# haotiansun14/rl-rep

Measured on AMD Instinct MI355X. Metric: gradient steps/sec (encoder+critic+actor) at batch=256, higher is better.
Workload: dtype f32

## Files before the change

rlrep_amd/csrc/engine.hip:

```cpp
#include "engine_internal.h"
#include <cstdarg>
#include <memory>

static thread_local char g_err[512] = "";
long long g_rl_launches = 0;
void rl_set_error(const char* fmt, ...) {
    va_list ap; va_start(ap, fmt); vsnprintf(g_err, sizeof(g_err), fmt, ap); va_end(ap);
}

static thread_local RlGrp g_grp;
static thread_local bool g_grp_on = false;
extern "C" const RlGrp* rl_grp_active() { return g_grp_on ? &g_grp : nullptr; }
struct GrpScope {
    bool set = false, prev_on = false; RlGrp prev{};
    explicit GrpScope(const rlrep_agent* ag) {
        if (!ag || ag->members <= 0) return;
        prev = g_grp; prev_on = g_grp_on;
        g_grp.members = ag->members; g_grp.stride = ag->grp_stride; g_grp.ring_stride = ag->grp_ring_stride; g_grp.seeds = ag->grp_seeds;
        g_grp_on = set = true;
    }
    ~GrpScope() { if (set) { g_grp = prev; g_grp_on = prev_on; } }
};
#define GROUP_REFUSE(what) \
    if (ag && ag->members > 0) { rl_set_error("%s: not available on a seed group (rlrep_group_create)", what); return RLREP_ERR_ARG; }
// ... 658 lines not shown
    };

    const std::vector<FinTask> cfins = {
        Builder::fin_sum(part_q + 0, nblk, 4, 1.0f / (float)B, ag->metrics + M_Q1_LOSS), Builder::fin_sum(part_q + 1, nblk, 4, 1.0f / (float)B, ag->metrics + M_Q2_LOSS),
        Builder::fin_sum(part_q + 2, nblk, 4, 1.0f / (float)B, ag->metrics + M_Q1), Builder::fin_sum(part_q + 3, nblk, 4, 1.0f / (float)B, ag->metrics + M_Q2)};
    const int ncdw_splits = rl_nc_dw_splits(B, F, H, 2);
    float* const ncdw_slab = ws.f((size_t)2 * ncdw_splits * H * F);
    float* const ncdw_bslab = ws.f((size_t)2 * ncdw_splits * H);
    const bool ncdw_in_adam = rl_nc_dw_engine() == 1 && ag->h.world_size <= 1 && ((H * F) & 3) == 0 && (H & 3) == 0 && ncdw_splits <= 16 && !rl_off("fold_ncdw");
    if (ncdw_in_adam) {
        const LT& w1 = ag->L.get("critic.l1.weight"); const LT& b1 = ag->L.get("critic.l1.bias");
        AdamTask::Slab sw; memset(&sw, 0, sizeof(sw));
        sw.off = w1.off - ag->L.group_off[1]; sw.n = 2ll * H * F; sw.per = (long long)H * F; sw.slab = ncdw_slab; sw.splits = ncdw_splits;
        AdamTask::Slab sb = sw;
        sb.off = b1.off - ag->L.group_off[1]; sb.n = 2ll * H; sb.per = H; sb.slab = ncdw_bslab;
        b.group_slabs[1] = {sw, sb};
    }
    auto critic_program = [&](Program& p, int hoist) {
        GemmTask tt[3], tn[3], tp[3];
        gauss_tasks(ag, !nft, fnet, s0.XF, SA, SA, gt, tt);
        gauss_tasks(ag, !nft, fnet, s0.XF2, SA, SA, gn, tn);
        gauss_tasks(ag, !nft, fnet, s0.XFpi, SA, SA, gp, tp);
        if (hoist == 2) {
            b.fwd_stage(p, {tt[0], tn[0], tp[0]}, "ft.l1(s,a) ft.l1(s',a') ft.l1(s,a_pi)");
            b.fwd_stage(p, {tt[1], tn[1], tp[1]}, "ft.l2 x3");
            b.fwd_stage(p, {tt[2], tn[2], tp[2]}, "ft.heads x3");
        } else if (hoist == 1) {
            b.fwd_stage(p, {actor_l(ag, 0, s0.XF2, SA, ab), actor_l(ag, 0, s0.XFpi, SA, ab_pi), tt[0]}, "actor.l1(s') actor.l1(s) ft.l1(s,a)");
            b.fwd_stage(p, {actor_l(ag, 1, nullptr, 0, ab), actor_l(ag, 1, nullptr, 0, ab_pi), tt[1]}, "actor.l2 x2 ft.l2");
            b.fwd_stage(p, {policy_head_task(ag, ab, s0.XF2 + S, SA, FLAG_DYN_EPS), policy_head_task(ag, ab_pi, s0.XFpi + S, SA, FLAG_DYN_EPS2), tt[2]},
                        "actor.head x2 ft.heads + policy");
            b.fwd_stage(p, {tn[0], tp[0]}, "ft.l1(s',a') ft.l1(s,a_pi)");
            b.fwd_stage(p, {tn[1], tp[1]}, "ft.l2 x2");
            b.fwd_stage(p, {tn[2], tp[2]}, "ft.heads x2");
        } else {
            b.fwd_stage(p, {actor_l(ag, 0, s0.XF2, SA, ab), tt[0]}, "actor.l1(s') ft.l1(s,a)");
            b.fwd_stage(p, {actor_l(ag, 1, nullptr, 0, ab), tt[1]}, "actor.l2 ft.l2");
            actor_head_stage(b, p, ag, ab, s0.XF2 + S, SA, {tt[2]}, "actor.head ft.heads + policy");
            b.fwd_stage(p, {tn[0]}, "ft.l1(s',a')");
            b.fwd_stage(p, {tn[1]}, "ft.l2");
            b.fwd_stage(p, {tn[2]}, "ft.heads");
        }
        {
            NcFwdTask live1 = nc_task(gt.HH, Pw("critic.l1.weight"), Pw("critic.l1.bias"), HmC, U, ag->W3("critic.l1.weight"));
            live1.sigma_out = SIG;
            nc_stage(p, {nc_task(gn.HH, Tw("critic_target.l1.weight"), Tw("critic_target.l1.bias"), HmT, nullptr, ag->W3("critic_target.l1.weight")),
                         nc_task(gn.HH, Tw("critic_target.l4.weight"), Tw("critic_target.l4.bias"), HmT + BH, nullptr, ag->W3("critic_target.l4.weight")),
                         live1,
                         nc_task(gt.HH, Pw("critic.l4.weight"), Pw("critic.l4.bias"), HmC + BH, U + BNH, ag->W3("critic.l4.weight"))}, "noise critic l1/l4 (target+live)");
        }
        b.fwd_stage(p, {Builder::fwd(HmT, H, B, H, Tw("critic_target.l2.weight"), H, Tw("critic_target.l2.bias"), H, Et, H, ACT_ELU),
                        Builder::fwd(HmT + BH, H, B, H, Tw("critic_target.l5.weight"), H, Tw("critic_target.l5.bias"), H, Et + BH, H, ACT_ELU),
                        Builder::fwd(HmC, H, B, H, Pw("critic.l2.weight"), H, Pw("critic.l2.bias"), H, Ec, H, ACT_ELU),
                        Builder::fwd(HmC + BH, H, B, H, Pw("critic.l5.weight"), H, Pw("critic.l5.bias"), H, Ec + BH, H, ACT_ELU)}, "critic l2/l5");
        QHeadCritic q; memset(&q, 0, sizeof(q));
        q.Et[0] = Et; q.Et[1] = Et + BH; q.Ec[0] = Ec; q.Ec[1] = Ec + BH;
        q.wt[0] = q.wt[1] = Tw("critic_target.l3.weight"); q.bt[0] = q.bt[1] = Tw("critic_target.l3.bias");
        q.wc[0] = q.wc[1] = Pw("critic.l3.weight"); q.bc[0] = q.bc[1] = Pw("critic.l3.bias");
        q.logp = ab.logp; q.R = s0.R; q.D = s0.D; q.alpha_state = ag->a.alpha_state_dev; q.gamma = ag->h.discount;
        q.inv_batch = ag->inv_batch(); q.dq = dq; q.GE[0] = GE; q.GE[1] = GE + BH; q.partial = part_q;
        q.B = B; q.H = H; q.nblk = nblk; q.train = 1; q.step = ag->adam_step + 1;
        p.stages.push_back({[=](hipStream_t st) { return rl_launch_qhead_critic(&q, st); }, "qhead critic"});
        b.dx_stage(p, {Builder::dx(GE, H, B, H, Pw("critic.l2.weight"), H, GHm, H, H, ACT_NONE, nullptr, 0),
                       Builder::dx(GE + BH, H, B, H, Pw("critic.l5.weight"), H, GHm + BH, H, H, ACT_NONE, nullptr, 0)}, "critic l2/l5 dx");
        b.dw_stage(p, {Builder::dw(dq, 1, 1, Ec, H, H, 2 * B, Gw("critic.l3.weight"), H, Gw("critic.l3.bias")),
                       Builder::dw(GE, H, H, HmC, H, H, B, Gw("critic.l2.weight"), H, Gw("critic.l2.bias")),
                       Builder::dw(GE + BH, H, H, HmC + BH, H, H, B, Gw("critic.l5.weight"), H, Gw("critic.l5.bias"))}, "critic dW l3 l2 l5");
        {
            NcDwBatch nb; memset(&nb, 0, sizeof(nb));
            nb.ntasks = 2;
            nb.lean = b.low_prio ? 1 : 0;
            int base_tile = 0;
            auto ncdw = [&](int q, float* Ubuf, float* GH, float* gW, float* gb) {
                NcDwTask& t = nb.t[q];
                t.U = Ubuf; t.GH = GH; t.ldgh = H; t.mean = gt.HH; t.sigma = SIG; t.ld_ml = 2 * F;
                t.noise = noise; t.gW = gW; t.gb = gb; t.B = B; t.F = F; t.H = H; t.N = N;
                t.tiles_k = (F + 31) / 32; t.ntiles = ((H + 15) / 16) * t.tiles_k; t.tile_base = base_tile; base_tile += t.ntiles;
            };
            ncdw(0, U, GHm, Gw("critic.l1.weight"), Gw("critic.l1.bias"));
            ncdw(1, U + BNH, GHm + BH, Gw("critic.l4.weight"), Gw("critic.l4.bias"));
            nb.splits = ncdw_splits; nb.slab = ncdw_slab; nb.bslab = ncdw_bslab;
            nb.engine = rl_nc_dw_engine();
            nb.fin_in_adam = ncdw_in_adam ? 1 : 0;
            if (nb.engine == 1) {
                base_tile = 0;
                for (int q = 0; q < 2; ++q) {
                    nb.t[q].ntiles = ((H + 63) / 64) * ((F + 63) / 64) * nb.splits; nb.t[q].tile_base = base_tile; base_tile += nb.t[q].ntiles;
                }
            }
            const int total = base_tile;
            p.stages.push_back({[=](hipStream_t st) { return rl_launch_nc_dw(&nb, total, st); }, "noise critic dW l1/l4"});
            Builder::tag(p, RLREP_ENGINE_NOISE_CRITIC, 2.0 * 2.0 * (double)B * N * F * H, 2.0 * 4.0 * ((double)B * N * H + (double)B * H + 2.0 * (double)B * F + (double)F * H));
        }
    };
    critic_program(ag->critic_bwd, 0);
    if (can_hoist) critic_program(ag->critic_bwd_h, 1);
    if (!ag->feat_bwd_h.stages.empty()) critic_program(ag->critic_bwd_h2, 2);
    b.adam(ag->critic_apply, 1, ag->h.lr_critic, nullptr, 0, 0, 0.f, cfins, "adam critic");
    critic_apply_folded(b, ag, "critic_target.l1.weight", cfins);

    auto actor_program = [&](Program& p, int& resume) {
        GemmTask tt[3];
        gauss_tasks(ag, !nft, fnet, s0.XFpi, SA, SA, gp, tt);
        b.fwd_stage(p, {actor_l(ag, 0, s0.XFpi, SA, ab_pi)}, "actor.l1(s)");
        b.fwd_stage(p, {actor_l(ag, 1, nullptr, 0, ab_pi)}, "actor.l2");
        actor_head_stage(b, p, ag, ab_pi, s0.XFpi + S, SA, {}, "actor.head + policy");
        b.fwd_stage(p, {tt[0]}, "ft.l1(s,a_pi)");
        b.fwd_stage(p, {tt[1]}, "ft.l2");
        b.fwd_stage(p, {tt[2]}, "ft.heads");
        resume = (int)p.stages.size();
        nc_stage(p, {nc_task(gp.HH, Pw("critic.l1.weight"), Pw("critic.l1.bias"), HmC, U, ag->W3("critic.l1.weight")),
                     nc_task(gp.HH, Pw("critic.l4.weight"), Pw("critic.l4.bias"), HmC + BH, U + BNH, ag->W3("critic.l4.weight"))}, "noise critic l1/l4");
        b.fwd_stage(p, {Builder::fwd(HmC, H, B, H, Pw("critic.l2.weight"), H, Pw("critic.l2.bias"), H, Ec, H, ACT_ELU),
                        Builder::fwd(HmC + BH, H, B, H, Pw("critic.l5.weight"), H, Pw("critic.l5.bias"), H, Ec + BH, H, ACT_ELU)}, "critic l2/l5");
        QHeadActor q; memset(&q, 0, sizeof(q));
        q.Ec[0] = Ec; q.Ec[1] = Ec + BH; q.wc[0] = q.wc[1] = Pw("critic.l3.weight"); q.bc[0] = q.bc[1] = Pw("critic.l3.bias");
        q.logp = ab_pi.logp; q.alpha_state = ag->a.alpha_state_dev; q.inv_batch = ag->inv_batch(); q.target_entropy = ag->h.target_entropy;
        q.GE[0] = GE; q.GE[1] = GE + BH; q.partial_loss = part_l; q.partial_c = ag->Gtail();
        q.B = B; q.H = H; q.nblk = nblk; q.step = ag->adam_step + 2;
        p.stages.push_back({[=](hipStream_t st) { return rl_launch_qhead_actor(&q, st); }, "qhead actor"});
        b.dx_stage(p, {Builder::dx(GE, H, B, H, Pw("critic.l2.weight"), H, GHm, H, H, ACT_NONE, nullptr, 0),
                       Builder::dx(GE + BH, H, B, H, Pw("critic.l5.weight"), H, GHm + BH, H, H, ACT_NONE, nullptr, 0)}, "critic l2/l5 dx");
        {
            NcDxTask t; memset(&t, 0, sizeof(t));
            t.GH[0] = GHm; t.GH[1] = GHm + BH; t.ldgh = H; t.U[0] = U; t.U[1] = U + BNH;
            t.W[0] = Pw("critic.l1.weight"); t.W[1] = Pw("critic.l4.weight"); t.noise = noise;
            t.lstd = gp.HH ? gp.HH + F : nullptr; t.ld_l = 2 * F; t.G = GTH; t.ldg = 2 * F;
            t.B = B; t.F = F; t.H = H; t.N = N; t.nheads = 2;
            t.tiles_k = (F + 63) / 64; t.ntiles = ((B + 3) / 4) * t.tiles_k; t.tile_base = 0;
            p.stages.push_back({[=](hipStream_t st) { return rl_launch_nc_dx(&t, st); }, "noise critic dX -> (dmean, dlog_std)"});
            Builder::tag(p, RLREP_ENGINE_NOISE_CRITIC, 2.0 * 2.0 * (double)B * N * F * H, 4.0 * (2.0 * ((double)B * N * H + (double)B * H + (double)F * H) + 3.0 * (double)B * F));
        }
        b.dx_stage(p, {Builder::dx(GTH, 2 * F, B, 2 * F, FT("mean_linear.weight"), Hv, GT2, Hv, Hv, ACT_RELU, gp.H2, Hv)}, "ft.heads dx");
        b.dx_stage(p, {Builder::dx(GT2, Hv, B, Hv, FT("l2.weight"), Hv, GT1, Hv, Hv, ACT_RELU, gp.H1, Hv)}, "ft.l2 dx");
        actor_backward(b, p, ag, ab_pi, s0.XFpi, SA, s0.XFpi + S, SA, Builder::dx(GT1, Hv, B, Hv, FT("l1.weight") ? FT("l1.weight") + S : nullptr, SA, ab_pi.dA, A, A, ACT_NONE, nullptr, 0));
    };
    actor_program(ag->actor_bwd, ag->actor_resume);
    actor_apply_program(b, ag, part_l, nblk);
    update_target_program(ag, "critic.l1.weight", "critic_target.l1.weight");

    for (int set = 0; set < rlrep_agent::NSETS; ++set) {
        const LT& f0 = ag->L.get(fnet + ".l1.weight");
        const LT& fl = ag->L.get(fnet + ".log_std_linear.bias");
        float* fbase = nft ? ag->a.param_dev : ag->a.target_dev;
        const Slot keep = defer_begin(b, ag, set, nft ? "f." : "f_target.", nft ? "f.l1.weight" : "f_target.l1.weight", fbase ? fbase + f0.off : nullptr,
                                      fl.off + fl.rows - f0.off);
        {
            rlrep_agent::DeferSet& D = ag->dset[set];
            const LT& p0 = ag->L.get("f.l1.weight");
            D.block_off = p0.off - ag->L.group_off[0]; D.block_n = fl.off + fl.rows - f0.off; D.block_which = nft ? 0 : 1;
            if (rl_off("fold_snapshot")) D.block_which = -1;
        }
        critic_program(ag->dset[set].critic_bwd, can_hoist ? 1 : 0);
        actor_program(ag->dset[set].actor_bwd, ag->dset[set].actor_resume);
        if (!can_hoist) ag->dset[set].actor_resume = 0;
        defer_end(b, ag, set, keep, "critic_target.l1.weight", cfins);
    }
}

Slot defer_begin(Builder& b, rlrep_agent* ag, int set, const char* prefix, const char* first, const float* block_src, int64_t block_n) {
    Workspace& ws = b.ws;
    const int B = ag->B, S = ag->d.state_dim, A = ag->d.action_dim, SA = S + A;
    Slot& s0 = ag->slot[0];
    rlrep_agent::DeferSet& D = ag->dset[set];
    Slot d; d.XE = nullptr; d.XF = ws.f((size_t)B * SA); d.XF2 = ws.f((size_t)B * SA); d.XFpi = ws.f((size_t)B * SA); d.R = ws.f(B); d.D = ws.f(B);
    D.slot = d;
// ... 1108 lines not shown
```

rlrep_amd/csrc/kparams.h:

```cpp
#pragma once
#include <stdint.h>
#include "dp_pull.h"
struct GroupCfg;

struct SlotFill {
    const float* ring; const int* idx;
    const float *s, *a, *r, *s2, *d;
    int B, S, A;
    float *XE, *XF, *XF2, *XFpi, *R, *D;
};

struct SelectAct {
    const float* obs; float* act;
    const float *W1, *b1, *W2, *b2, *W3, *b3;
    int S, Ha, A, explore;
    float lo, hi;
    unsigned long long seed, offset;
};
struct PhiloxFill {
    float* dst_f; int* dst_i; long long n;
    int kind;
    float std; int hi; const int* hi_dev;
    unsigned long long seed, offset; const int* step_dev; uint32_t stream_id;
    int step_add;
// ... 86 lines not shown
    if (g.in_a) g.in_a = (const float*)((uintptr_t)g.in_a + (uintptr_t)mdelta);
    if (g.in_b) g.in_b = (const float*)((uintptr_t)g.in_b + (uintptr_t)mdelta);
    if (g.alpha_state) g.alpha_state = (double*)((uintptr_t)g.alpha_state + (uintptr_t)mdelta);
    return g;
}
template <bool GRP = false>
__device__ inline void finalize_tasks(const FinTask* __restrict__ fin, int nfin, int lane, const DpPull* dp = nullptr, long long mdelta = 0) {
    for (int q = 0; q < nfin; ++q) {
        const FinTask f = fin_record<GRP>(fin[q], mdelta);
        if (f.kind == FIN_SUM) {
            float s = 0.f;
            for (int i = lane; i < f.count; i += 64) s += f.partials[(size_t)i * f.stride];
            s = wave_sum(s);
            if (lane == 0) *f.out = s * f.scale;
        } else if (f.kind == FIN_COMBINE) {
            if (lane == 0) *f.out = f.scale * (*f.in_a) + f.scale_b * (*f.in_b);
        } else if (f.kind == FIN_INC) {
            if (lane == 0) *reinterpret_cast<int*>(f.out) += 1;
        } else if (f.kind == FIN_COPY) {
            if (lane == 0) *f.out = *f.in_a;
        } else if (f.kind == FIN_ALPHA) {
            float s = 0.f;
            if (dp) {
                const long long toff = (long long)(f.partials - dp->base[dp->rank]);
                for (int i = lane; i < f.count; i += 64) s += dp_sum1(*dp, toff + (long long)i * f.stride);
            } else {
                for (int i = lane; i < f.count; i += 64) s += f.partials[(size_t)i * f.stride];
            }
            s = wave_sum(s);
            if (lane == 0) {
                double* st = f.alpha_state;
                const float mean_c = s * f.scale;
                const double alpha = exp(st[0]);
                *f.out = (float)alpha * mean_c;
                if (f.learn) {
                    const double g = (double)mean_c * alpha;
                    const double b1 = (double)f.beta1, b2 = (double)f.beta2;
                    st[3] += 1.0;
                    st[1] = st[1] + (1.0 - b1) * (g - st[1]);
                    st[2] = st[2] * b2 + (1.0 - b2) * g * g;
                    const double bc1 = 1.0 - pow(b1, st[3]), bc2 = 1.0 - pow(b2, st[3]);
                    const double denom = sqrt(st[2]) / sqrt(bc2) + (double)f.eps;
                    st[0] = st[0] - ((double)f.lr / bc1) * (st[1] / denom);
                }
                *f.out2 = (float)exp(st[0]);
            }
        } else if (f.kind == FIN_HISTORY) {
            __builtin_amdgcn_s_waitcnt(0x0F70);
            asm volatile("" ::: "memory");
            int* seq = reinterpret_cast<int*>(const_cast<float*>(f.partials));
            const int n = *seq;
            float* rec = f.out + (size_t)(n % f.count) * RL_HIST_REC;
            if (lane < f.stride) rec[lane] = __hip_atomic_load(f.in_a + lane, __ATOMIC_RELAXED, __HIP_MEMORY_SCOPE_AGENT);
            if (lane == RL_HIST_TAG) reinterpret_cast<int*>(rec)[RL_HIST_TAG] = n;
            if (lane == 0) *seq = n + 1;
        }
    }
}
#endif

struct NcFwdTask {
    const float* mean; const float* lstd; int ld_ml;
    const float* noise;
    const float* W; const float* bias;
    const unsigned char* W3;
    float* Hm;
    float* U;
    float* sigma_out;
    int B, F, H, N;
    int tiles_h, tile_base, ntiles;
};

#define NC_MAX_TASKS 4
struct NcFwdBatch { int ntasks; int engine; int cols; int nt_u; NcFwdTask t[NC_MAX_TASKS]; };

struct NcDwTask {
    const float* U; const float* GH; int ldgh;
    const float* mean; const float* sigma; int ld_ml;
    const float* noise;
    float* gW; float* gb;
    int B, F, H, N;
    int tiles_k, tile_base, ntiles;
};
struct NcDwBatch { int ntasks; int lean; int engine; int splits; float* slab; float* bslab; int fin_in_adam; int pad_; NcDwTask t[2]; };

struct NcDxTask {
    const float* GH[2]; int ldgh;
    const float* U[2];
    const float* W[2];
    const float* noise;
    const float* lstd; int ld_l;
    float* G; int ldg;
    int B, F, H, N, nheads;
    int tiles_k, tile_base, ntiles;
};


#define NC_NF_HOST 5

struct InfoNce {
    float* S; int ldS;
    int ncols, diag_off;
    const float* rhat; const float* r; float* drhat;
    float* partial; int B, nblk; float inv_batch; GroupCfg* step;
    const float* Z; int ldZ, F; const float* theta_w; const float* theta_b;
    const float* ZM; int ldZM;
};
struct ColSum { const float* X; int ldX; const float* w; float* out; int rows, F; const float* X2; int ldX2; const float* w2; float* out2; float* outb2; int rows2; DpSlots dp; };
#define RL_SLOTS_MAX_F 65536
struct SpederRows {
    const float* phi; const float* mu; const float* mu_r; const float* phibar;
    const float* theta_w; const float* theta_b; const float* r;
    float* c; float* drhat; float* partial; int B, F, nblk; float inv_batch; GroupCfg* step;
};
struct SpederGrads {
    const float* phi; const float* mu; const float* c; const float* drhat; const float* phibar; const float* v;
    const float* theta_w; float* Gphi; float* Gmu; int B, F; float inv_batch;
};
struct RegStats { const float* X[4]; const float* C[4]; int B, H, nbc, nbr; float lambda; float* partial; };

struct DiffsrPerturb {
    const float* alphabars; const int* idx; const float* s2; int ld_s2; const float* eps;
    float* XN; float* TGT; int B, S; GroupCfg* step0; GroupCfg* step1;
};
struct DiffsrScore {
    float* U; const float* PHI; const float* TGT; const float* alphabars; const int* idx;
    float* GPHI; float* partial; int B, F, S; float sigma, inv_batch;
};

enum XcKind : int { XC_GEMM = 0, XC_HEADS_VAE = 1, XC_QHEAD_CRITIC = 2, XC_QHEAD_ACTOR = 3 };
struct XcPhase {
    int kind;
    int task0, ntasks;
    int la, lb, vecA, vecB, pre;
    int tiles;
    int aux;
    int dyn;
    int rbg, R;
    int tb[GEMM_MAX_TASKS], tcs[GEMM_MAX_TASKS];
};
#define XC_GROUPS 8
#define XC_FLAG_STRIDE 64
struct XcLaunch {
    const XcPhase* ph; int nph;
    const GemmTask* tasks; const HeadsVae* hv; const QHeadCritic* qc; const QHeadActor* qa;
    int ntasks, nhv, nqc, nqa;
    unsigned* flags;
    unsigned* err;
    int rbg;
    int mpg;
    const float* dyn[3];
    int low_prio;
};
```

rlrep_amd/csrc/noisecritic.hip:

```cpp
#include <type_traits>
#include "common.h"
extern long long g_rl_launches;
#include "kparams.h"
#include "x3.h"

#define NC_NF 5

extern __shared__ __attribute__((aligned(16))) float nc_smem[];

#ifdef RL_TIMING_NC
__device__ unsigned long long g_nc_tim[6 * 4096];
extern "C" int rl_nc_timing_fetch(unsigned long long* host, int n) {
    return (int)hipMemcpyFromSymbol(host, HIP_SYMBOL(g_nc_tim), sizeof(unsigned long long) * n);
}
#define NCT(k) do { if (threadIdx.x == 0 && blockIdx.x < 4096) g_nc_tim[6 * blockIdx.x + (k)] = (k) < 4 ? clock64() : wall_clock64(); } while (0)
#else
#define NCT(k) do {} while (0)
#endif

__device__ __forceinline__ void ld4(const float* p, bool vec, int valid, float (&v)[4]) {
    if (vec && valid == 4) { f32x4 x = *reinterpret_cast<const f32x4*>(p); v[0] = x[0]; v[1] = x[1]; v[2] = x[2]; v[3] = x[3]; }
    else {
#pragma unroll
        for (int s = 0; s < 4; ++s) v[s] = (s < valid) ? p[s] : 0.f;
// ... 1182 lines not shown
            }
            if (want_bias) asum += (o.a[0] + o.a[1]) + (o.a[2] + o.a[3]);
        };
        const int nchunks = (Mb + 15) / 16;
        const int ngroups = (nchunks + 31) / 32;
        auto compg = [&](int g, const Chunk (&S)[4]) {
            const int c = w + 32 * g;
            Prep p0, p1;
            prep(c, S[0], p0);
            __builtin_amdgcn_sched_barrier(0);
            prep(c + 8, S[1], p1); mac(p0);
            __builtin_amdgcn_sched_barrier(0);
            prep(c + 16, S[2], p0); mac(p1);
            __builtin_amdgcn_sched_barrier(0);
            prep(c + 24, S[3], p1); mac(p0);
            __builtin_amdgcn_sched_barrier(0);
            mac(p1);
        };
        if constexpr (LEAN) {
            for (int g = 0; g < ngroups; g += 2) {
                __builtin_amdgcn_sched_barrier(0);
                if (g + 2 < ngroups) {
                    compg(g, S0);     loadg(g + 2, S0); __builtin_amdgcn_sched_barrier(0);
                    compg(g + 1, S1); loadg(g + 3, S1);
                } else {
                    compg(g, S0);
                    if (g + 1 < ngroups) compg(g + 1, S1);
                }
            }
        } else
        for (int g = 0; g < ngroups; g += 4) {
            __builtin_amdgcn_sched_barrier(0);
            if (g + 4 < ngroups) {
                compg(g, S0);     loadg(g + 4, S0); __builtin_amdgcn_sched_barrier(0);
                compg(g + 1, S1); loadg(g + 5, S1); __builtin_amdgcn_sched_barrier(0);
                compg(g + 2, S2); loadg(g + 6, S2); __builtin_amdgcn_sched_barrier(0);
                compg(g + 3, S3); loadg(g + 7, S3);
            } else {
                compg(g, S0);
                if (g + 1 < ngroups) compg(g + 1, S1);
                if (g + 2 < ngroups) compg(g + 2, S2);
                if (g + 3 < ngroups) compg(g + 3, S3);
            }
        }
    }
#pragma unroll
    for (int f = 0; f < 2; ++f)
#pragma unroll
        for (int r = 0; r < 4; ++r) red[w][f][r][lane] = acc[f][r];
    if (want_bias) {
        asum += __shfl_xor(asum, 16, 64);
        asum += __shfl_xor(asum, 32, 64);
        if (lane < 16) bsum[w][lane] = asum;
    }
    __syncthreads();
    {
        const int ol = threadIdx.x & 63, q = threadIdx.x >> 6;
        const int f = q >> 2, r = q & 3;
        float v = 0.f;
#pragma unroll
        for (int ww = 0; ww < 8; ++ww) v += red[ww][f][r][ol];
        const int row = j0 + (ol >> 4) * 4 + r, colk = k0 + 16 * f + (ol & 15);
        if (row < H && colk < F) {
            const size_t o = (size_t)row * F + colk;
            t.gW[o] = v;
        }
    }
    if (want_bias && threadIdx.x < 16 && j0 + (int)threadIdx.x < H) {
        float v = 0.f;
#pragma unroll
        for (int ww = 0; ww < 8; ++ww) v += bsum[ww][threadIdx.x];
        t.gb[j0 + threadIdx.x] = v;
    }
}

#define NDW_IMGB (64 * NX_RSB)
#define NDW_OPB (3 * NDW_IMGB)
#define NDW_BUFB (2 * NDW_OPB)

template <int OFF> __device__ __forceinline__ void ndw_fload_at(u32x4 (&d)[3], unsigned addr) {
    nx_read<OFF>(d[0], addr); nx_read<OFF + NDW_IMGB>(d[1], addr); nx_read<OFF + 2 * NDW_IMGB>(d[2], addr);
}

__global__ __launch_bounds__(512) void nc_dw_x3_kernel(NcDwBatch nb) {
    __shared__ __attribute__((aligned(16))) unsigned char L[2 * NDW_BUFB];
    const int bid = blockIdx.x;
    const int q = (nb.ntasks > 1 && bid >= nb.t[1].tile_base) ? 1 : 0;
    const NcDwTask& t = nb.t[q];
    const int F = t.F, H = t.H, B = t.B;
    constexpr int N = 4 * NC_NF;
    const int TK = (F + 63) >> 6, TJ = (H + 63) >> 6;
    int local = bid - t.tile_base;
    {
        const int ngrp = TJ * nb.splits;
        if ((ngrp & 7) == 0 && (t.tile_base & 7) == 0) {
            const int x = local & 7, y = local >> 3;
            local = ((y / TK) * 8 + x) * TK + (y % TK);
        }
    }
    const int sp = local / (TJ * TK); local -= sp * (TJ * TK);
    const int tj = local / TK, tk = local - tj * TK;
    const int j0 = tj * 64, k0 = tk * 64;
    const int bs = (B + nb.splits - 1) / nb.splits;
    const int bbeg = min(sp * bs, B), nbr = min(bs, B - bbeg);
    const int nrows = N * nbr;
    const int S = (nrows + 31) >> 5;
    const int w8 = threadIdx.x >> 6;
    float* const slab = nb.slab + ((size_t)(q * nb.splits + sp) * H) * F;
    if (nbr <= 0) {
        for (int e = threadIdx.x; e < 64 * 64; e += 512) {
            const int jj = j0 + (e >> 6), kk = k0 + (e & 63);
            if (jj < H && kk < F) slab[(size_t)jj * F + kk] = 0.f;
        }
        if (tk == 0 && threadIdx.x < 64 && j0 + (int)threadIdx.x < H) nb.bslab[(size_t)(q * nb.splits + sp) * H + j0 + threadIdx.x] = 0.f;
        return;
    }

    if (w8 >= 4) {
        const int tid = threadIdx.x - 256;
        const int c = tid & 63, rq = tid >> 6;
        const int j = min(j0 + c, H - 1), k = min(k0 + c, F - 1);
        const float invN = 1.0f / (float)N;
        const float* const Uc = t.U + (size_t)bbeg * N * H + j;
        const float* const Gc = t.GH + (size_t)bbeg * t.ldgh + j;
        const float* const Mc = t.mean + (size_t)bbeg * t.ld_ml + k;
        const float* const Sc = t.sigma + (size_t)bbeg * F + k;
        const float* const Zc = t.noise + k;
        const int wofs = c * NX_RSB + rq * 16;
        struct PReg { float u[8], g[2], mu[2], sg[2], nz[8]; };
        auto gload = [&](int s, PReg& r) {
            const int r0 = 32 * min(s, S - 1) + 8 * rq;
#pragma unroll
            for (int h = 0; h < 2; ++h) {
                const int rg = min(r0 + 4 * h, nrows - 4);
                const int lb = rg / N, n0 = rg - lb * N;
                const float* up = Uc + (size_t)rg * H;
#pragma unroll
                for (int e = 0; e < 4; ++e) { r.u[4 * h + e] = up[(size_t)e * H]; r.nz[4 * h + e] = Zc[(size_t)(n0 + e) * F]; }
                r.g[h] = Gc[(size_t)lb * t.ldgh]; r.mu[h] = Mc[(size_t)lb * t.ld_ml]; r.sg[h] = Sc[(size_t)lb * F];
            }
        };
        float bsum = 0.f;
        auto produce = [&](int s, const PReg& r, unsigned char* buf) {
            const int r0 = 32 * s + 8 * rq;
            float a[8], x[8];
#pragma unroll
            for (int h = 0; h < 2; ++h) {
                const bool valid = r0 + 4 * h < nrows;
                const float g = valid ? r.g[h] * invN : 0.f, mu = valid ? r.mu[h] : 0.f, sg = valid ? r.sg[h] : 0.f;
#pragma unroll
                for (int e = 0; e < 4; ++e) {
                    a[4 * h + e] = g * fminf(r.u[4 * h + e] + 1.f, 1.f);
                    x[4 * h + e] = fmaf(sg, r.nz[4 * h + e], mu);
                    bsum += a[4 * h + e];
                }
            }
            u32x4 ah, am, al, xh, xm, xl;
#pragma unroll
            for (int p2 = 0; p2 < 4; ++p2) {
                unsigned h, m, l;
                x3_split2(a[2 * p2], a[2 * p2 + 1], h, m, l); ah[p2] = h; am[p2] = m; al[p2] = l;
                x3_split2(x[2 * p2], x[2 * p2 + 1], h, m, l); xh[p2] = h; xm[p2] = m; xl[p2] = l;
            }
            unsigned char* pa = buf + wofs;
            *reinterpret_cast<u32x4*>(pa) = ah;
            *reinterpret_cast<u32x4*>(pa + NDW_IMGB) = am;
            *reinterpret_cast<u32x4*>(pa + 2 * NDW_IMGB) = al;
            *reinterpret_cast<u32x4*>(pa + NDW_OPB) = xh;
            *reinterpret_cast<u32x4*>(pa + NDW_OPB + NDW_IMGB) = xm;
            *reinterpret_cast<u32x4*>(pa + NDW_OPB + 2 * NDW_IMGB) = xl;
        };
        PReg ra, rb;
        gload(0, ra); gload(1, rb);
        produce(0, ra, L);
        gload(2, ra);
        __syncthreads();
        for (int s = 0; s < S; s += 2) {
            if (s + 1 < S) produce(s + 1, rb, L + NDW_BUFB);
            gload(s + 3, rb);
            __syncthreads();
            if (s + 1 < S) {
                if (s + 2 < S) produce(s + 2, ra, L);
                gload(s + 4, ra);
                __syncthreads();
            }
        }
        float* const red = reinterpret_cast<float*>(L);
        __syncthreads();
        red[rq * 64 + c] = bsum;
        __syncthreads();
        if (tk == 0 && rq == 0 && j0 + c < H)
            nb.bslab[(size_t)(q * nb.splits + sp) * H + j0 + c] = ((red[c] + red[64 + c]) + red[128 + c]) + red[192 + c];
        return;
    }

    const int lane = threadIdx.x & 63, w = w8;
    const int m16 = lane & 15, kq = lane >> 4;
    const int wj = w >> 1, wk = w & 1;
    const unsigned lds0 = (unsigned)(uintptr_t)(__attribute__((address_space(3))) unsigned char*)L + (unsigned)(m16 * NX_RSB + kq * 16);
    const unsigned aofs = (unsigned)(32 * wj * NX_RSB), bofs = (unsigned)(NDW_OPB + 32 * wk * NX_RSB);
    f32x4 acc[2][2];
#pragma unroll
    for (int a = 0; a < 2; ++a)
#pragma unroll
        for (int b2 = 0; b2 < 2; ++b2) acc[a][b2] = (f32x4){0.f, 0.f, 0.f, 0.f};
    __syncthreads();
    for (int s = 0; s < S; ++s) {
        const unsigned base = lds0 + (unsigned)((s & 1) * NDW_BUFB);
        u32x4 fa[2][3], fb[2][3];
        ndw_fload_at<0>(fa[0], base + aofs);
        ndw_fload_at<0>(fb[0], base + bofs);
        ndw_fload_at<16 * NX_RSB>(fa[1], base + aofs);
        ndw_fload_at<16 * NX_RSB>(fb[1], base + bofs);
        asm volatile("s_waitcnt lgkmcnt(6)" : "+v"(fa[0][0]), "+v"(fa[0][1]), "+v"(fa[0][2]), "+v"(fb[0][0]), "+v"(fb[0][1]), "+v"(fb[0][2]));
#define NDW_MM(A, Bq)                                                                                                   \
        {                                                                                                               \
            const bf16x8 Ah = __builtin_bit_cast(bf16x8, fa[A][0]), Am = __builtin_bit_cast(bf16x8, fa[A][1]), Al = __builtin_bit_cast(bf16x8, fa[A][2]); \
            const bf16x8 Bh = __builtin_bit_cast(bf16x8, fb[Bq][0]), Bm = __builtin_bit_cast(bf16x8, fb[Bq][1]), Bl = __builtin_bit_cast(bf16x8, fb[Bq][2]); \
            f32x4 d = acc[A][Bq];                                                                                       \
            d = __builtin_amdgcn_mfma_f32_16x16x32_bf16(Al, Bh, d, 0, 0, 0);                                            \
            d = __builtin_amdgcn_mfma_f32_16x16x32_bf16(Ah, Bl, d, 0, 0, 0);                                            \
            d = __builtin_amdgcn_mfma_f32_16x16x32_bf16(Am, Bm, d, 0, 0, 0);                                            \
            d = __builtin_amdgcn_mfma_f32_16x16x32_bf16(Am, Bh, d, 0, 0, 0);                                            \
            d = __builtin_amdgcn_mfma_f32_16x16x32_bf16(Ah, Bm, d, 0, 0, 0);                                            \
            d = __builtin_amdgcn_mfma_f32_16x16x32_bf16(Ah, Bh, d, 0, 0, 0);                                            \
            acc[A][Bq] = d;                                                                                             \
        }
        NDW_MM(0, 0)
        asm volatile("s_waitcnt lgkmcnt(0)" : "+v"(fa[1][0]), "+v"(fa[1][1]), "+v"(fa[1][2]), "+v"(fb[1][0]), "+v"(fb[1][1]), "+v"(fb[1][2]));
        NDW_MM(0, 1) NDW_MM(1, 0) NDW_MM(1, 1)
#undef NDW_MM
        __syncthreads();
    }
    __syncthreads();
    __syncthreads();
#pragma unroll
    for (int a = 0; a < 2; ++a)
#pragma unroll
        for (int b2 = 0; b2 < 2; ++b2) {
            const int kk = k0 + 32 * wk + 16 * b2 + m16;
#pragma unroll
            for (int r = 0; r < 4; ++r) {
                const int jj = j0 + 32 * wj + 16 * a + 4 * kq + r;
                if (jj < H && kk < F) slab[(size_t)jj * F + kk] = acc[a][b2][r];
            }
        }
}

__global__ __launch_bounds__(256) void nc_dw_fin_kernel(NcDwBatch nb) {
    const int q = blockIdx.y;
    const NcDwTask& t = nb.t[q];
    const size_t HF = (size_t)t.H * t.F;
    const size_t e = (size_t)blockIdx.x * 256 + threadIdx.x;
    const float* s0 = nb.slab + (size_t)q * nb.splits * HF;
    if (e < HF) {
        float v = s0[e];
        for (int sp = 1; sp < nb.splits; ++sp) v += s0[(size_t)sp * HF + e];
        t.gW[e] = v;
    }
    if (e < (size_t)t.H) {
        const float* b0 = nb.bslab + (size_t)q * nb.splits * t.H;
        float v = b0[e];
        for (int sp = 1; sp < nb.splits; ++sp) v += b0[(size_t)sp * t.H + e];
        t.gb[e] = v;
    }
}

extern "C" int rl_nc_fwd_cols() { return 128; }
extern "C" void rl_nc_fwd_plan(const NcFwdTask* tasks, int ntasks, int* engine, int* g2, int* cols) {
    const int B = tasks[0].B, F = tasks[0].F, H = tasks[0].H;
    const bool want_x3 = !rl_off("x3");
    bool x3 = want_x3 && (F % 32) == 0 && F >= 64;
    for (int q = 0; q < ntasks; ++q) {
        const NcFwdTask& t = tasks[q];
        x3 = x3 && t.N == 4 * NC_NF && (t.ld_ml & 3) == 0 && t.F == F && t.H == H && t.B == B &&
             ((((uintptr_t)t.mean) | ((uintptr_t)t.lstd) | ((uintptr_t)t.noise) | ((uintptr_t)t.W) | ((uintptr_t)t.sigma_out)) & 15) == 0;
    }
    if (x3) {
        *engine = 1; *g2 = 2;
        const long long wg128 = (long long)ntasks * ((B + 7) / 8) * ((H + 127) / 128);
        *cols = wg128 >= 256 ? 128 : 64;
        return;
    }
    *engine = 0;
    *cols = rl_nc_fwd_cols();
    *g2 = ((long long)ntasks * ((B + 3) / 4) * ((H + 63) / 64) <= 2048) ? 1 : 2;
}
extern "C" int rl_launch_nc_fwd(const NcFwdBatch* nb, int total_tiles, int g2, hipStream_t st) {
    if (total_tiles <= 0) return 0;
    for (int q = 0; q < nb->ntasks; ++q) if (nb->t[q].N != 4 * NC_NF) return -2;
    const int F = nb->t[0].F, N = nb->t[0].N;
    if (nb->engine == 1) {
        if ((F % 32) != 0 || g2 != 2) return -3;
#ifdef RL_EXPERIMENTS
        const int wide = rl_off("nc_x3_wide") ? 0 : 1;
        const int quad = rl_off("nc_x3_q") ? 0 : 1;
        if (nb->cols == 128 && quad) hipLaunchKernelGGL(nc_fwd_x3q_kernel, dim3(total_tiles), dim3(256), 2 * NX_BUFB, st, *nb);
        else if (nb->cols == 128 && wide) hipLaunchKernelGGL((nc_fwd_x3w_kernel<8>), dim3(total_tiles), dim3(512), 2 * NX_BUFB, st, *nb);
        else if (nb->cols == 128) hipLaunchKernelGGL((nc_fwd_x3_kernel<2>), dim3(total_tiles), dim3(512), 2 * NX_BUFB, st, *nb);
#else
        if (nb->cols == 128) hipLaunchKernelGGL(nc_fwd_x3q_kernel, dim3(total_tiles), dim3(256), 2 * NX_BUFB, st, *nb);
#endif
        else hipLaunchKernelGGL((nc_fwd_x3_kernel<1>), dim3(total_tiles), dim3(512), 2 * NX_BUFB, st, *nb);
        return (int)hipGetLastError();
    }
    const int Fp = (F + 15) & ~15;
    const size_t lds = (size_t)(8 * g2 + N) * (Fp + 16) * sizeof(float);
    const int nw = nb->cols / 16;
    if (nw == 8) {
        if (g2 == 1) hipLaunchKernelGGL((nc_fwd_kernel<1, 8>), dim3(total_tiles), dim3(512), lds, st, *nb);
        else if (g2 == 2) hipLaunchKernelGGL((nc_fwd_kernel<2, 8>), dim3(total_tiles), dim3(512), lds, st, *nb);
        else hipLaunchKernelGGL((nc_fwd_kernel<4, 8>), dim3(total_tiles), dim3(512), lds, st, *nb);
    } else {
        if (g2 == 1) hipLaunchKernelGGL((nc_fwd_kernel<1, 4>), dim3(total_tiles), dim3(256), lds, st, *nb);
        else if (g2 == 2) hipLaunchKernelGGL((nc_fwd_kernel<2, 4>), dim3(total_tiles), dim3(256), lds, st, *nb);
        else hipLaunchKernelGGL((nc_fwd_kernel<4, 4>), dim3(total_tiles), dim3(256), lds, st, *nb);
    }
    return (int)hipGetLastError();
}

extern "C" int rl_nc_dx_engine(const NcDxTask* t) {
    if (rl_off("x3")) return 0;
    if (t->N != 4 * NC_NF || (t->H % 32) != 0 || (t->ldgh & 1) || t->nheads < 1 || t->nheads > 2 || t->tiles_k != (t->F + 63) / 64) return 0;
    for (int h = 0; h < t->nheads; ++h) if (((((uintptr_t)t->U[h]) | ((uintptr_t)t->GH[h])) & 7) != 0) return 0;
    return 1;
}
extern "C" int rl_launch_nc_dx(const NcDxTask* t, hipStream_t st) {
    if (t->ntiles <= 0) return 0;
    if (t->N != 4 * NC_NF) return -2;
    bool vec = ((t->H & 3) == 0) && ((t->ldgh & 3) == 0);
    for (int h = 0; h < t->nheads; ++h) vec = vec && ((((uintptr_t)t->U[h]) | ((uintptr_t)t->GH[h])) & 15) == 0;
    if (rl_nc_dx_engine(t) == 1) {
        hipLaunchKernelGGL(nc_dx_x3_kernel, dim3(t->ntiles), dim3(512), 0, st, *t);
        return (int)hipGetLastError();
    }
    if (vec) hipLaunchKernelGGL(nc_dx_kernel<true>, dim3(t->ntiles), dim3(512), 0, st, *t);
    else hipLaunchKernelGGL(nc_dx_kernel<false>, dim3(t->ntiles), dim3(512), 0, st, *t);
    return (int)hipGetLastError();
}

extern "C" int rl_nc_init() {
    const size_t lds = (size_t)NCDW_BB * (NCDW_TLD + 16) * sizeof(float);
    hipError_t e = hipSuccess;
#ifdef RL_EXPERIMENTS
    e = hipFuncSetAttribute((const void*)nc_fwd_x3_kernel<2>, hipFuncAttributeMaxDynamicSharedMemorySize, 2 * NX_BUFB);
    if (e == hipSuccess) e = hipFuncSetAttribute((const void*)nc_fwd_x3w_kernel<8>, hipFuncAttributeMaxDynamicSharedMemorySize, 2 * NX_BUFB);
#endif
    if (e == hipSuccess) e = hipFuncSetAttribute((const void*)nc_fwd_x3q_kernel, hipFuncAttributeMaxDynamicSharedMemorySize, 2 * NX_BUFB);
    if (e == hipSuccess) e = hipFuncSetAttribute((const void*)nc_fwd_x3_kernel<1>, hipFuncAttributeMaxDynamicSharedMemorySize, 2 * NX_BUFB);
    if (e != hipSuccess) return (int)e;
    if (e == hipSuccess) e = hipFuncSetAttribute((const void*)nc_dw_kernel<true>, hipFuncAttributeMaxDynamicSharedMemorySize, (int)lds);
    if (e != hipSuccess) return (int)e;
    return (int)hipFuncSetAttribute((const void*)nc_dw_kernel<false>, hipFuncAttributeMaxDynamicSharedMemorySize, (int)lds);
}

extern "C" int rl_nc_dw_engine() { return rl_off("x3") ? 0 : 1; }
extern "C" int rl_nc_dw_splits(int B, int F, int H, int ntasks) {
    const int tiles = ((H + 63) / 64) * ((F + 63) / 64) * ntasks;
    int sp = (256 + tiles - 1) / tiles;
    sp = sp < 1 ? 1 : sp > 16 ? 16 : sp;
    const int maxsp = (B + 7) / 8;
    return sp > maxsp ? (maxsp < 1 ? 1 : maxsp) : sp;
}
extern "C" int rl_launch_nc_dw(const NcDwBatch* nb, int total_tiles, hipStream_t st) {
    if (total_tiles <= 0) return 0;
    for (int q = 0; q < nb->ntasks; ++q) if (nb->t[q].N != 4 * NC_NF || nb->t[q].B <= 0) return -2;
    if (nb->engine == 1) {
        if (!nb->slab || !nb->bslab || nb->splits < 1) return -3;
        const NcDwTask& t0 = nb->t[0];
        for (int q = 1; q < nb->ntasks; ++q) if (nb->t[q].H != t0.H || nb->t[q].F != t0.F || nb->t[q].B != t0.B) return -3;
        hipLaunchKernelGGL(nc_dw_x3_kernel, dim3(total_tiles), dim3(512), 0, st, *nb);
        if (nb->fin_in_adam) return (int)hipGetLastError();
        const size_t HF = (size_t)t0.H * t0.F;
        hipLaunchKernelGGL(nc_dw_fin_kernel, dim3((unsigned)((HF + 255) / 256), nb->ntasks), dim3(256), 0, st, *nb);
        ++g_rl_launches;
        return (int)hipGetLastError();
    }
    const size_t lds = (size_t)NCDW_BB * (NCDW_TLD + 16) * sizeof(float);
    if (nb->lean) hipLaunchKernelGGL(nc_dw_kernel<true>, dim3(total_tiles), dim3(512), lds, st, *nb);
    else hipLaunchKernelGGL(nc_dw_kernel<false>, dim3(total_tiles), dim3(512), lds, st, *nb);
    return (int)hipGetLastError();
}
```

Measured before the change: 3983.

## Move noise-critic dW x-operand production into MFMA waves with software pipelining

In the x3 noise-critic weight-gradient kernel, the producer waves (4-7) previously loaded mean, sigma and noise, built x = mu + sigma*z, split it into bf16 triples and wrote both operands to LDS. A new templated path moves the x-operand work onto the MFMA waves (0-3). Those waves prefetch x inputs two steps ahead into registers and write the next buffer between MFMA steps, which halves the producers' per-step work and balances load across waves. This costs extra registers and global loads on the MFMA waves and adds a more intricate double-buffer schedule. It can be disabled with the ncdw_cx switch.

Result: no change. 3987, median of 6 (+0.1%).

```diff
diff --git a/rlrep_amd/csrc/engine.hip b/rlrep_amd/csrc/engine.hip
--- a/rlrep_amd/csrc/engine.hip
+++ b/rlrep_amd/csrc/engine.hip
@@ -764,6 +764,7 @@
             nb.splits = ncdw_splits; nb.slab = ncdw_slab; nb.bslab = ncdw_bslab;
             nb.engine = rl_nc_dw_engine();
             nb.fin_in_adam = ncdw_in_adam ? 1 : 0;
+            nb.split_x = rl_off("ncdw_cx") ? 0 : 1;
             if (nb.engine == 1) {
                 base_tile = 0;
                 for (int q = 0; q < 2; ++q) {
diff --git a/rlrep_amd/csrc/kparams.h b/rlrep_amd/csrc/kparams.h
--- a/rlrep_amd/csrc/kparams.h
+++ b/rlrep_amd/csrc/kparams.h
@@ -192,7 +192,7 @@
     int B, F, H, N;
     int tiles_k, tile_base, ntiles;
 };
-struct NcDwBatch { int ntasks; int lean; int engine; int splits; float* slab; float* bslab; int fin_in_adam; int pad_; NcDwTask t[2]; };
+struct NcDwBatch { int ntasks; int lean; int engine; int splits; float* slab; float* bslab; int fin_in_adam; int split_x; NcDwTask t[2]; };
 
 struct NcDxTask {
     const float* GH[2]; int ldgh;
diff --git a/rlrep_amd/csrc/noisecritic.hip b/rlrep_amd/csrc/noisecritic.hip
--- a/rlrep_amd/csrc/noisecritic.hip
+++ b/rlrep_amd/csrc/noisecritic.hip
@@ -1288,6 +1288,7 @@
     nx_read<OFF>(d[0], addr); nx_read<OFF + NDW_IMGB>(d[1], addr); nx_read<OFF + 2 * NDW_IMGB>(d[2], addr);
 }
 
+template <bool SX>
 __global__ __launch_bounds__(512) void nc_dw_x3_kernel(NcDwBatch nb) {
     __shared__ __attribute__((aligned(16))) unsigned char L[2 * NDW_BUFB];
     const int bid = blockIdx.x;
@@ -1312,6 +1313,12 @@
     const int nrows = N * nbr;
     const int S = (nrows + 31) >> 5;
     const int w8 = threadIdx.x >> 6;
+    const int c = threadIdx.x & 63, rq = (threadIdx.x >> 6) & 3;
+    const int k = min(k0 + c, F - 1);
+    const float* const Mc = t.mean + (size_t)bbeg * t.ld_ml + k;
+    const float* const Sc = t.sigma + (size_t)bbeg * F + k;
+    const float* const Zc = t.noise + k;
+    const int wofs = c * NX_RSB + rq * 16;
     float* const slab = nb.slab + ((size_t)(q * nb.splits + sp) * H) * F;
     if (nbr <= 0) {
         for (int e = threadIdx.x; e < 64 * 64; e += 512) {
@@ -1321,18 +1328,45 @@
         if (tk == 0 && threadIdx.x < 64 && j0 + (int)threadIdx.x < H) nb.bslab[(size_t)(q * nb.splits + sp) * H + j0 + threadIdx.x] = 0.f;
         return;
     }
+    struct XReg { float mu[2], sg[2], nz[8]; };
+    auto xload = [&](int s, XReg& r) {
+        const int r0 = 32 * min(s, S - 1) + 8 * rq;
+#pragma unroll
+        for (int h = 0; h < 2; ++h) {
+            const int rg = min(r0 + 4 * h, nrows - 4);
+            const int lb = rg / N, n0 = rg - lb * N;
+#pragma unroll
+            for (int e = 0; e < 4; ++e) r.nz[4 * h + e] = Zc[(size_t)(n0 + e) * F];
+            r.mu[h] = Mc[(size_t)lb * t.ld_ml]; r.sg[h] = Sc[(size_t)lb * F];
+        }
+    };
+    auto xproduce = [&](int s, const XReg& r, unsigned char* buf) {
+        const int r0 = 32 * s + 8 * rq;
+        float x[8];
+#pragma unroll
+        for (int h = 0; h < 2; ++h) {
+            const bool valid = r0 + 4 * h < nrows;
+            const float mu = valid ? r.mu[h] : 0.f, sg = valid ? r.sg[h] : 0.f;
+#pragma unroll
+            for (int e = 0; e < 4; ++e) x[4 * h + e] = fmaf(sg, r.nz[4 * h + e], mu);
+        }
+        u32x4 xh, xm, xl;
+#pragma unroll
+        for (int p2 = 0; p2 < 4; ++p2) {
+            unsigned h, m, l;
+            x3_split2(x[2 * p2], x[2 * p2 + 1], h, m, l); xh[p2] = h; xm[p2] = m; xl[p2] = l;
+        }
+        unsigned char* pa = buf + wofs + NDW_OPB;
+        *reinterpret_cast<u32x4*>(pa) = xh;
+        *reinterpret_cast<u32x4*>(pa + NDW_IMGB) = xm;
+        *reinterpret_cast<u32x4*>(pa + 2 * NDW_IMGB) = xl;
+    };
 
     if (w8 >= 4) {
-        const int tid = threadIdx.x - 256;
-        const int c = tid & 63, rq = tid >> 6;
-        const int j = min(j0 + c, H - 1), k = min(k0 + c, F - 1);
+        const int j = min(j0 + c, H - 1);
         const float invN = 1.0f / (float)N;
         const float* const Uc = t.U + (size_t)bbeg * N * H + j;
         const float* const Gc = t.GH + (size_t)bbeg * t.ldgh + j;
-        const float* const Mc = t.mean + (size_t)bbeg * t.ld_ml + k;
-        const float* const Sc = t.sigma + (size_t)bbeg * F + k;
-        const float* const Zc = t.noise + k;
-        const int wofs = c * NX_RSB + rq * 16;
         struct PReg { float u[8], g[2], mu[2], sg[2], nz[8]; };
         auto gload = [&](int s, PReg& r) {
             const int r0 = 32 * min(s, S - 1) + 8 * rq;
@@ -1342,8 +1376,9 @@
                 const int lb = rg / N, n0 = rg - lb * N;
                 const float* up = Uc + (size_t)rg * H;
 #pragma unroll
-                for (int e = 0; e < 4; ++e) { r.u[4 * h + e] = up[(size_t)e * H]; r.nz[4 * h + e] = Zc[(size_t)(n0 + e) * F]; }
-                r.g[h] = Gc[(size_t)lb * t.ldgh]; r.mu[h] = Mc[(size_t)lb * t.ld_ml]; r.sg[h] = Sc[(size_t)lb * F];
+                for (int e = 0; e < 4; ++e) { r.u[4 * h + e] = up[(size_t)e * H]; if (!SX) r.nz[4 * h + e] = Zc[(size_t)(n0 + e) * F]; }
+                r.g[h] = Gc[(size_t)lb * t.ldgh];
+                if (!SX) { r.mu[h] = Mc[(size_t)lb * t.ld_ml]; r.sg[h] = Sc[(size_t)lb * F]; }
             }
         };
         float bsum = 0.f;
@@ -1353,11 +1388,11 @@
 #pragma unroll
             for (int h = 0; h < 2; ++h) {
                 const bool valid = r0 + 4 * h < nrows;
-                const float g = valid ? r.g[h] * invN : 0.f, mu = valid ? r.mu[h] : 0.f, sg = valid ? r.sg[h] : 0.f;
+                const float g = valid ? r.g[h] * invN : 0.f, mu = (valid && !SX) ? r.mu[h] : 0.f, sg = (valid && !SX) ? r.sg[h] : 0.f;
 #pragma unroll
                 for (int e = 0; e < 4; ++e) {
                     a[4 * h + e] = g * fminf(r.u[4 * h + e] + 1.f, 1.f);
-                    x[4 * h + e] = fmaf(sg, r.nz[4 * h + e], mu);
+                    if (!SX) x[4 * h + e] = fmaf(sg, r.nz[4 * h + e], mu);
                     bsum += a[4 * h + e];
                 }
             }
@@ -1366,15 +1401,17 @@
             for (int p2 = 0; p2 < 4; ++p2) {
                 unsigned h, m, l;
                 x3_split2(a[2 * p2], a[2 * p2 + 1], h, m, l); ah[p2] = h; am[p2] = m; al[p2] = l;
-                x3_split2(x[2 * p2], x[2 * p2 + 1], h, m, l); xh[p2] = h; xm[p2] = m; xl[p2] = l;
+                if (!SX) { x3_split2(x[2 * p2], x[2 * p2 + 1], h, m, l); xh[p2] = h; xm[p2] = m; xl[p2] = l; }
             }
             unsigned char* pa = buf + wofs;
             *reinterpret_cast<u32x4*>(pa) = ah;
             *reinterpret_cast<u32x4*>(pa + NDW_IMGB) = am;
             *reinterpret_cast<u32x4*>(pa + 2 * NDW_IMGB) = al;
-            *reinterpret_cast<u32x4*>(pa + NDW_OPB) = xh;
-            *reinterpret_cast<u32x4*>(pa + NDW_OPB + NDW_IMGB) = xm;
-            *reinterpret_cast<u32x4*>(pa + NDW_OPB + 2 * NDW_IMGB) = xl;
+            if (!SX) {
+                *reinterpret_cast<u32x4*>(pa + NDW_OPB) = xh;
+                *reinterpret_cast<u32x4*>(pa + NDW_OPB + NDW_IMGB) = xm;
+                *reinterpret_cast<u32x4*>(pa + NDW_OPB + 2 * NDW_IMGB) = xl;
+            }
         };
         PReg ra, rb;
         gload(0, ra); gload(1, rb);
@@ -1410,8 +1447,7 @@
     for (int a = 0; a < 2; ++a)
 #pragma unroll
         for (int b2 = 0; b2 < 2; ++b2) acc[a][b2] = (f32x4){0.f, 0.f, 0.f, 0.f};
-    __syncthreads();
-    for (int s = 0; s < S; ++s) {
+    auto mstep = [&](int s) {
         const unsigned base = lds0 + (unsigned)((s & 1) * NDW_BUFB);
         u32x4 fa[2][3], fb[2][3];
         ndw_fload_at<0>(fa[0], base + aofs);
@@ -1436,7 +1472,31 @@
         asm volatile("s_waitcnt lgkmcnt(0)" : "+v"(fa[1][0]), "+v"(fa[1][1]), "+v"(fa[1][2]), "+v"(fb[1][0]), "+v"(fb[1][1]), "+v"(fb[1][2]));
         NDW_MM(0, 1) NDW_MM(1, 0) NDW_MM(1, 1)
 #undef NDW_MM
+    };
+    if (SX) {
+        XReg xa, xb;
+        xload(0, xa); xload(1, xb);
+        xproduce(0, xa, L);
+        xload(2, xa);
         __syncthreads();
+        for (int s = 0; s < S; s += 2) {
+            mstep(s);
+            xproduce(s + 1, xb, L + NDW_BUFB);
+            xload(s + 3, xb);
+            __syncthreads();
+            if (s + 1 < S) {
+                mstep(s + 1);
+                xproduce(s + 2, xa, L);
+                xload(s + 4, xa);
+                __syncthreads();
+            }
+        }
+    } else {
+        __syncthreads();
+        for (int s = 0; s < S; ++s) {
+            mstep(s);
+            __syncthreads();
+        }
     }
     __syncthreads();
     __syncthreads();
@@ -1575,7 +1635,8 @@
         if (!nb->slab || !nb->bslab || nb->splits < 1) return -3;
         const NcDwTask& t0 = nb->t[0];
         for (int q = 1; q < nb->ntasks; ++q) if (nb->t[q].H != t0.H || nb->t[q].F != t0.F || nb->t[q].B != t0.B) return -3;
-        hipLaunchKernelGGL(nc_dw_x3_kernel, dim3(total_tiles), dim3(512), 0, st, *nb);
+        if (nb->split_x) hipLaunchKernelGGL(nc_dw_x3_kernel<true>, dim3(total_tiles), dim3(512), 0, st, *nb);
+        else hipLaunchKernelGGL(nc_dw_x3_kernel<false>, dim3(total_tiles), dim3(512), 0, st, *nb);
         if (nb->fin_in_adam) return (int)hipGetLastError();
         const size_t HF = (size_t)t0.H * t0.F;
         hipLaunchKernelGGL(nc_dw_fin_kernel, dim3((unsigned)((HF + 255) / 256), nb->ntasks), dim3(256), 0, st, *nb);
```
